# david-cortes/cmfrec

Measured on AMD Instinct MI355X. Metric: ALS rows/sec ((users+items)/iteration time), implicit ALS-CG k=50 fp64, higher is better.
Workload: dtype f64

## Files before the change

### cmfrec_amd/csrc/cg_kernels.hpp

```cpp
#pragma once
#include <hip/hip_runtime.h>
#include <stdint.h>
#include <type_traits>

#include "lanes.hpp"

namespace cmfhip {

constexpr int WAVE = 64;
constexpr int TILE = 64;
constexpr int MAX_W = 8;
#ifndef CMF_CG_WAVES_PER_SIMD
#define CMF_CG_WAVES_PER_SIMD 2
#endif
#ifndef CMF_CG_WAVES_PER_SIMD_F32
#define CMF_CG_WAVES_PER_SIMD_F32 3
#endif
#ifndef CMF_CG_WAVES_PER_SIMD_LOW
#define CMF_CG_WAVES_PER_SIMD_LOW 3
#endif
constexpr int CG_NTSEL_MAX_S = 7;
template <typename T, int W, int NRES_, int NTSEL = 0> constexpr int cg_waves_per_simd()
{
    if (sizeof(T) == 8 && NTSEL == 1 && W <= 8) return CMF_CG_WAVES_PER_SIMD_LOW;
// ... 52 lines not shown
    const T *values;
    const T *bias_sub;
    const T *weights = nullptr;
    const T *wsum = nullptr;
    const int *order;
    const RowDesc *desc;
    int nrows;
    const T *BtB;
    T lam, lam_last;
    int scale_lam, scale_bias_const;
    int max_cg_steps;
    int precond;
    int koff = 0, kc = 0;
    const T *CtC = nullptr;
    const T *UC = nullptr;
    T w_side = 0;
    int rows_with_u = 0;
    int row_first = 0;
    const size_t *indptr2 = nullptr;
    const int *indices2 = nullptr;
    const T *values2 = nullptr;
    const T *C2 = nullptr;
    int *counter = nullptr;
    int p_side = 0, scale_lam_sideinfo = 0;
    const T *Bi = nullptr;
    const T *BiTBi = nullptr;
    int ki = 0;
    T w_imp = 0;
    const T *rconst = nullptr;
    size_t ldr = 0;
    int gx = 0;
#ifdef CMF_CG_DEBUG
    int dbg = 0;
#endif
#ifdef CMF_CG_TICKS
    unsigned long long *ticks = nullptr;
#endif
};
#ifdef CMF_CG_TICKS
#define CMF_TICK() __builtin_amdgcn_s_memtime()
__device__ __forceinline__ void cg_ticks_flush(unsigned long long *t, int slot, unsigned long long wait, unsigned long long pass, unsigned long long rows,
                                               unsigned long long total, int lane)
{
    if (t != nullptr && lane == 0) {
        atomicAdd(t + 4 * slot + 0, wait); atomicAdd(t + 4 * slot + 1, pass); atomicAdd(t + 4 * slot + 2, rows); atomicAdd(t + 4 * slot + 3, total);
    }
// ... 889 lines not shown
{
    static_assert(NE == 4 || NE == 2 || NE == 0, "entries per lane group");
    constexpr bool MIX = NE == 0;
    static_assert(!MIX || CMF_TINY_WAVES_PER_SIMD >= 3, "the mixed launch lives in the dynamically scheduled loop");
    using Tile = typename TinyTile<T, S, (NE == 2) ? 2 : 4>::type;
    constexpr bool GRAM = IMPLICIT || GRAMX;
    extern __shared__ __attribute__((aligned(16))) unsigned char smem_raw[];
    T *G = reinterpret_cast<T *>(smem_raw);
    constexpr bool PV = pass_vector_in_lds<T>();
    __shared__ __attribute__((aligned(16))) T s_pv[PV ? 4 : 1][PV ? 64 : 1];
    const int tid = threadIdx.x;
    const int lane = tid & 63;
    auto short_row = [&](int nnz_) -> bool { return MIX && nnz_ <= 16; };
    auto entry_of = [&](int nnz_) -> int { return (NE == 2 || short_row(nnz_)) ? (lane >> 2) : (lane >> 1); };
    const int k = P.k;
    constexpr bool GREG = tiny_greg<T, GRAM>();
    constexpr int GR = GREG ? gram_rows<T>(S) : 8;
    if (GRAM) {
        stage_gramian<T, S, GR>(G, P.BtB, k, tid, blockDim.x);
        __syncthreads();
    }
    GramRegs<T, GREG ? S : 1, GREG ? GR : 8> greg;
    if constexpr (GREG) greg.load(G, lane);
    const int nwaves = gridDim.x * 4;
    struct Pre { int idx; T x; T a; T g; };
    auto load_desc = [&](int rix_) -> RowDesc {
        RowDesc d; d.row = 0; d.nnz = 0; d.st = 0;
        if (rix_ < P.nrows) d = P.desc[rix_];
        d.row = __builtin_amdgcn_readfirstlane(d.row);
        d.nnz = __builtin_amdgcn_readfirstlane(d.nnz);
        d.st = ((unsigned long long)(unsigned)__builtin_amdgcn_readfirstlane((int)(d.st >> 32)) << 32) |
               (unsigned)__builtin_amdgcn_readfirstlane((int)(d.st & 0xffffffffu));
        return d;
    };
    auto load_pre = [&](const RowDesc &d) -> Pre {
        Pre q; q.idx = 0; q.x = T(0); q.a = T(0); q.g = T(1);
        const int ent = entry_of(d.nnz);
        if (ent < d.nnz) {
            const size_t pos = d.st + (size_t)ent;
            q.idx = P.indices[pos];
            q.x = P.values[pos];
            q.g = entry_weight<T, IMPLICIT>(P, pos);
            if (!IMPLICIT && P.bias_sub != nullptr) q.x -= P.bias_sub[q.idx];
        }
        if (d.nnz > 0 && lane < k) q.a = P.A[(size_t)d.row * P.lda + lane];
        return q;
    };
// ... 47 lines not shown
        if (GRAMX && P.rconst != nullptr && lane < k) r_d += P.rconst[(size_t)d.row * P.ldr + lane];
        if (lane >= k) r_d = T(0);
        T p_d = r_d;
        T r_old = wave_sum(r_d * r_d);
        bool done = (r_old <= (T)1e-12);
        for (int step = 0; step < P.max_cg_steps && !done; step++) {
            T Ap_d = run_pass(p_d, std::integral_constant<int, 1>{});
            Ap_d += lam * p_d;
            if (!IMPLICIT && lam != lam_last && lane == k - 1) Ap_d += (lam_last - lam) * p_d;
            if (lane >= k) Ap_d = T(0);
            T alpha = cg_div(r_old, wave_sum(Ap_d * p_d));
            a_d += alpha * p_d;
            r_d -= alpha * Ap_d;
            T r_new = wave_sum(r_d * r_d);
            if (r_new <= (T)1e-8) done = true;
            else {
                p_d = p_d * cg_div(r_new, r_old) + r_d;
                r_old = r_new;
            }
        }
        if (lane < k) P.A[(size_t)d.row * P.lda + lane] = a_d;
    };

    int rix = blockIdx.x * 4 + (tid >> 6);
#if CMF_TINY_WAVES_PER_SIMD >= 3
    {
        const int cslot = rix % CG_NCOUNTERS;
        int *const my_counter = P.counter + cslot * CG_COUNTER_STRIDE;
        const int cbase = nwaves + cslot;
        auto issue_claim = [&]() -> int {
            int v = 0;
            if (lane == 0) v = atomicAdd(my_counter, 1);
            return v;
        };
        const int c1 = issue_claim(), c2 = issue_claim();
        int rnxt = cbase + CG_NCOUNTERS * __builtin_amdgcn_readfirstlane(c1);
        int rnn = cbase + CG_NCOUNTERS * __builtin_amdgcn_readfirstlane(c2);
        RowDesc d0 = load_desc(rix), d1 = load_desc(rnxt);
        Pre p0 = load_pre(d0);
        Tile tA;
        int pend = issue_claim();
        while (rix < P.nrows) {
            const bool shrt = short_row(d0.nnz);
            if (CMF_DBG(P, 1)) {
                dbg_fill_tile<(NE == 2) ? 2 : 4, S>(tA, (T)(p0.idx & 3) * (T)0.001);
            } else if constexpr (MIX) {
                if (shrt) load_tile2<T, S>(tA, P.B, P.ldb, k, p0.idx, d0.nnz, lane);
// ... 505 lines not shown
```

### cmfrec_amd/csrc/device.hpp

```cpp
#pragma once
#include <hip/hip_runtime.h>
#include <algorithm>
#include <cstdio>
#include <cstdlib>
#include <cstring>
#include <numeric>
#include <string>
#include <vector>

#include "../../include/cmfrec_hip.h"
#include "device_base.hpp"
#include "cg_kernels.hpp"
#include "chol_kernels.hpp"
#include "dense_kernels.hpp"
#include "gram_cg_kernels.hpp"
#include "topn_kernels.hpp"

namespace cmfhip {

constexpr int MAX_DEVICES = 16;
constexpr int NBINS = 6;
constexpr int BIN_VHEAVY = 0;
constexpr int BIN_HEAVY = 1;
constexpr int BIN_MED4 = 2;
// ... 198 lines not shown
            sl_vrow.upload(s_row.data(), s_row.size(), st);
            sl_first.upload(s_first.data(), s_first.size(), st);
            sl_count.upload(s_count.data(), s_count.size(), st);
            row_sl_off.upload(s_off.data(), s_off.size(), st);
            h_row_sl_off = s_off;
            gram_part.alloc((size_t)n_slices * GRAM_PART);
        }
        HIP_CHECK(hipStreamSynchronize(st));
    }
};

struct DeviceInfo {
    int device = 0;
    int num_cus = 256;
    hipStream_t stream = nullptr;
    DevBuf<real_t> cg_gfull, cg_rconst;
    DevBuf<real_t> tile_init;
    DevBuf<int> row_counter;
    DevBuf<real_t> potrs_inv, potrs_tmp;
    DevBuf<real_t> potrs_ref;
    DevBuf<real_t> gemm_ws;
    hipStream_t aux_stream = nullptr;
    hipEvent_t fork_ev = nullptr, join_ev = nullptr;
    hipStream_t eig_stream_ = nullptr;
    hipEvent_t eig_fork = nullptr;
    hipStream_t eig_stream()
    {
        if (!eig_stream_) HIP_CHECK(hipStreamCreateWithFlags(&eig_stream_, hipStreamNonBlocking));
        return eig_stream_;
    }
    mutable bool nonneg_now = false;
    mutable int max_cd_steps = 100;
    mutable real_t l1_now = 0;
    mutable real_t l1_last_now = 0;
    mutable real_t l1_scale = 1;
    DeviceInfo() = default;
    DeviceInfo(const DeviceInfo &) = delete;
    DeviceInfo &operator=(const DeviceInfo &) = delete;
    ~DeviceInfo()
    {
        if (eig_fork) (void)hipEventDestroy(eig_fork);
        if (eig_stream_) (void)hipStreamDestroy(eig_stream_);
        if (fork_ev) (void)hipEventDestroy(fork_ev);
        if (join_ev) (void)hipEventDestroy(join_ev);
        for (int i = 0; i < MAX_BIN_STREAMS; i++) {
            if (bin_join[i]) (void)hipEventDestroy(bin_join[i]);
            if (i > 0 && bin_streams[i]) (void)hipStreamDestroy(bin_streams[i]);
        }
        if (aux_stream) (void)hipStreamDestroy(aux_stream);
        if (stream) (void)hipStreamDestroy(stream);
    }
    void ensure_aux()
    {
        if (aux_stream) return;
        HIP_CHECK(hipStreamCreateWithFlags(&aux_stream, hipStreamNonBlocking));
        HIP_CHECK(hipEventCreateWithFlags(&fork_ev, hipEventDisableTiming));
        HIP_CHECK(hipEventCreateWithFlags(&join_ev, hipEventDisableTiming));
    }
    static constexpr int MAX_BIN_STREAMS = 5;
    hipStream_t bin_streams[MAX_BIN_STREAMS] = {nullptr, nullptr, nullptr, nullptr, nullptr};
    hipEvent_t bin_join[MAX_BIN_STREAMS] = {nullptr, nullptr, nullptr, nullptr, nullptr};
    void ensure_bin_streams(int n)
    {
        ensure_aux();
        bin_streams[0] = aux_stream;
        if (!bin_join[0]) HIP_CHECK(hipEventCreateWithFlags(&bin_join[0], hipEventDisableTiming));
        for (int i = 1; i < n && i < MAX_BIN_STREAMS; i++) {
            if (!bin_streams[i]) HIP_CHECK(hipStreamCreateWithFlags(&bin_streams[i], hipStreamNonBlocking));
            if (!bin_join[i]) HIP_CHECK(hipEventCreateWithFlags(&bin_join[i], hipEventDisableTiming));
        }
    }
};

struct EventPair { hipEvent_t a, b; };
struct BinTimers {
    std::vector<EventPair> ev[NBINS];
    void clear()
    {
        for (auto &v : ev) {
            for (auto &p : v) { (void)hipEventDestroy(p.a); (void)hipEventDestroy(p.b); }
// ... 43 lines not shown
    if (k <= 64) {
        int nblocks = std::max(1, std::min(dev.num_cus * 2, (n + 127) / 128));
        int rpb = (n + nblocks - 1) / nblocks;
        nblocks = (n + rpb - 1) / rpb;
        if (nblocks < 1) nblocks = 1;
        size_t need = (size_t)nblocks * k * k;
        if (ws.partial.n < need) ws.partial.alloc(need);
        const int rem = (sizeof(real_t) == 8 && k > 48 && k <= 52) ? k - 48 : 0;
        switch (rem) {
#define CMF_GRAM_REM(R) case R: hipLaunchKernelGGL((gram_mfma_partial_kernel<real_t, R>), dim3(nblocks), dim3(256), 0, dev.stream, B, ldb, n, k, rpb, ws.partial.ptr); break;
            CMF_GRAM_REM(1) CMF_GRAM_REM(2) CMF_GRAM_REM(3) CMF_GRAM_REM(4)
#undef CMF_GRAM_REM
            default: hipLaunchKernelGGL((gram_mfma_partial_kernel<real_t, 0>), dim3(nblocks), dim3(256), 0, dev.stream, B, ldb, n, k, rpb, ws.partial.ptr); break;
        }
        hipLaunchKernelGGL(gram_reduce_kernel<real_t>, dim3((k * k + GRAM_RED_ENT - 1) / GRAM_RED_ENT), dim3(256), 0, dev.stream,
                           ws.partial.ptr, nblocks, k * k, out, scale, add_diag, k);
    } else {
        launch_gemm<true>(dev, k, k, n, scale, B, ldb, B, ldb, out, (size_t)k);
        if (add_diag != 0)
            hipLaunchKernelGGL(add_diag_kernel<real_t>, dim3((k + 255) / 256), dim3(256), 0, dev.stream, out, k, 0, k, add_diag);
    }
    HIP_CHECK(hipGetLastError());
}

struct CgCall {
    real_t *A; size_t lda;
    const real_t *B; size_t ldb;
    int k;
    const real_t *bias_sub;
    const real_t *BtB;
    real_t lam, lam_last;
    bool scale_lam, scale_bias_const;
    int max_cg_steps;
    bool implicit;
    bool precond = false;
    int koff = 0, kc = 0;
    const real_t *CtC = nullptr, *UC = nullptr;
    real_t w_side = 0;
    int rows_with_u = 0, p_side = 0;
    bool scale_lam_sideinfo = false;
    const SparseShard *X2 = nullptr;
    const real_t *C2 = nullptr;
    const real_t *Bi = nullptr, *BiTBi = nullptr;
    int ki = 0;
    real_t w_imp = 0;
    const real_t *gsum = nullptr;
    int skip_first = 0;
    const real_t *Gx = nullptr, *rconst_x = nullptr;
    size_t ldr_x = 0;
    const real_t *values_override = nullptr, *weights_override = nullptr;
    bool gx_all_rows = false;
    const real_t *wsum_override = nullptr;
};

enum class CgVariant { Auto, Generic };
CgVariant cg_variant_from_env();

constexpr int NCOUNTER_SETS = 2 * NBINS + 2;
constexpr size_t ROW_COUNTER_INTS = 64 + (size_t)NCOUNTER_SETS * CG_NCOUNTERS * CG_COUNTER_STRIDE;
inline size_t cg_counter_offset(int bin) { return 64 + (size_t)bin * CG_NCOUNTERS * CG_COUNTER_STRIDE; }

__global__ void __launch_bounds__(256) poison_lds_kernel(int words)
{
    extern __shared__ unsigned int poison_words[];
    volatile unsigned int *w = poison_words;
    for (int e = threadIdx.x; e < words; e += 256) w[e] = 0xFFFFFFFFu;
}
inline void poison_lds(hipStream_t st, int num_cus)
{
    if (!switches().poison_lds) return;
    constexpr int BYTES = 80 * 1024;
    static thread_local bool attr_set = false;
    if (!attr_set) {
        HIP_CHECK(hipFuncSetAttribute((const void *)poison_lds_kernel, hipFuncAttributeMaxDynamicSharedMemorySize, BYTES));
        attr_set = true;
// ... 20 lines not shown
    constexpr int threads = 64 * W * RPB;
    size_t smem = (((IMPLICIT || GRAMX) ? (size_t)gram_elems<real_t>(S) : 0) + (size_t)RPB * 2 * W * 64) * sizeof(real_t);
    auto kern = cg_rows_kernel<real_t, S, IMPLICIT, W, RPB, GRAMX, NRES_, NTSEL>;
    static thread_local int bpc_dev[MAX_DEVICES] = {0};
    int &blocks_per_cu = bpc_dev[std::min(std::max(dev.device, 0), MAX_DEVICES - 1)];
    if (blocks_per_cu == 0) {
        if (smem > 48 * 1024)
            HIP_CHECK(hipFuncSetAttribute((const void *)kern, hipFuncAttributeMaxDynamicSharedMemorySize, (int)smem));
        int nb = 0;
        HIP_CHECK(hipOccupancyMaxActiveBlocksPerMultiprocessor(&nb, kern, threads, smem));
        blocks_per_cu = std::max(1, nb);
    }
    int teams_needed = (count + RPB - 1) / RPB;
    int grid = std::min(teams_needed, dev.num_cus * blocks_per_cu);
    hipLaunchKernelGGL(kern, dim3(grid), dim3(threads), smem, st, P);
    HIP_CHECK(hipGetLastError());
    if (tm) {
        HIP_CHECK(hipEventRecord(ev.b, st));
        tm->ev[bin].push_back(ev);
    }
}

template <int S, bool IMPLICIT, bool GRAMX = false>
inline void launch_cg_tiny(const DeviceInfo &dev, CgParams<real_t> P, int first, int count, BinTimers *tm, hipStream_t st, int n_gt16)
{
    if (count <= 0) return;
    EventPair ev{nullptr, nullptr};
    if (tm) {
        HIP_CHECK(hipEventCreate(&ev.a));
        HIP_CHECK(hipEventCreate(&ev.b));
        HIP_CHECK(hipEventRecord(ev.a, st));
    }
    poison_lds(st, dev.num_cus);
    constexpr bool tiny16_on = true;
    const int count_le16 = std::min(count, std::max(0, first + count - std::max(first, n_gt16)));
    size_t smem = ((IMPLICIT || GRAMX) ? (size_t)gram_elems<real_t>(S) : 0) * sizeof(real_t);
    const int di = std::min(std::max(dev.device, 0), MAX_DEVICES - 1);
    CgParams<real_t> P1 = P;
    P1.order += first;
    P1.desc += first;
    P1.nrows = count;
    P1.counter = dev.row_counter.ptr + cg_counter_offset(BIN_TINY);
    {
        const bool mixed = tiny16_on && count_le16 > 0;
        auto kern = mixed ? cg_rows_tiny_kernel<real_t, S, IMPLICIT, GRAMX, 0> : cg_rows_tiny_kernel<real_t, S, IMPLICIT, GRAMX, 4>;
        static thread_local int bpc_dev[MAX_DEVICES][2] = {{0}};
        int &blocks_per_cu = bpc_dev[di][mixed ? 1 : 0];
        if (blocks_per_cu == 0) {
            int nb = 0;
            HIP_CHECK(hipOccupancyMaxActiveBlocksPerMultiprocessor(&nb, kern, 256, smem));
            blocks_per_cu = std::max(1, nb);
        }
        const int grid = std::min((count + 3) / 4, dev.num_cus * blocks_per_cu);
        hipLaunchKernelGGL(kern, dim3(grid), dim3(256), smem, st, P1);
    }
    HIP_CHECK(hipGetLastError());
    if (tm) {
        HIP_CHECK(hipEventRecord(ev.b, st));
        tm->ev[BIN_TINY].push_back(ev);
    }
}

void launch_gram_wave(dim3 grid, hipStream_t st, const CgParams<real_t> &P, const GramParams<real_t> &G, bool implicit, int rem);

template <bool GRAMX>
inline bool vh_takes_gram(int k, const SparseShard &X)
{
    if (GRAMX || k > 16 * GRAM_NTT) return false;
    return (switches().vh != 0) ? switches().vh == 2 : X.prefer_gram((size_t)k * sizeof(real_t));
}

template <int S, bool IMPLICIT, bool GRAMX = false>
inline void launch_cg_vheavy(const DeviceInfo &dev_, CgParams<real_t> P, const SparseShard &X, BinTimers *tm, hipStream_t st)
{
    const int nvh = X.bin_rows[BIN_VHEAVY];
    if (nvh <= 0) return;
    struct { hipStream_t stream; int num_cus; } dev{st, dev_.num_cus};
    EventPair ev{nullptr, nullptr};
    if (tm) {
        HIP_CHECK(hipEventCreate(&ev.a));
        HIP_CHECK(hipEventCreate(&ev.b));
        HIP_CHECK(hipEventRecord(ev.a, dev.stream));
    }
    if (vh_takes_gram<GRAMX>(P.k, X)) {
        GramParams<real_t> G;
        G.sl_vrow = X.sl_vrow.ptr; G.sl_first = X.sl_first.ptr; G.sl_count = X.sl_count.ptr; G.row_sl_off = X.row_sl_off.ptr;
        G.part = X.gram_part.ptr; G.n_slices = X.n_slices; G.nvh = nvh;
        P.nrows = nvh;
#ifdef CMF_CG_DEBUG
        if (switches().debug_ticks) {
            static unsigned long long *d_t = nullptr;
            unsigned long long h[4];
            if (d_t == nullptr) { HIP_CHECK(hipMalloc((void **)&d_t, sizeof(h))); HIP_CHECK(hipMemset(d_t, 0, sizeof(h))); }
            else {
                HIP_CHECK(hipDeviceSynchronize());
                HIP_CHECK(hipMemcpy(h, d_t, sizeof(h), hipMemcpyDeviceToHost));
                if (h[1] > 0)
                    fprintf(stderr, "gram_wave: %.0f ticks per wave, %llu waves, %llu slices, %llu nnz: %.1f ticks per nnz and wave\n",
                            (double)h[0] / h[1], h[1], h[2], h[3], (double)h[0] / (double)h[3]);
                HIP_CHECK(hipMemset(d_t, 0, sizeof(h)));
            }
            G.ticks = d_t;
        }
#endif
        poison_lds(dev.stream, dev.num_cus);
        const bool slice_kernel = switches().gram_slice;
        if (slice_kernel)
            hipLaunchKernelGGL((gram_slice_kernel<real_t, IMPLICIT>), dim3(std::min(X.n_slices, dev.num_cus * 2)), dim3(64 * GRAM_NW), 0,
                           dev.stream, P, G);
        else {
            const dim3 gw(std::min((X.n_slices + 3) / 4, dev.num_cus * 4));
            const int rem = (sizeof(real_t) == 8) ? P.k - 16 * (GRAM_NTT - 1) : 0;
            launch_gram_wave(gw, dev.stream, P, G, IMPLICIT, rem);
        }
        poison_lds(dev.stream, dev.num_cus);
        hipLaunchKernelGGL((gram_cg_kernel<real_t, IMPLICIT>), dim3(std::min(nvh, dev.num_cus * 8)), dim3(256), 0, dev.stream, P, G);
        HIP_CHECK(hipGetLastError());
        if (tm) {
            HIP_CHECK(hipEventRecord(ev.b, dev.stream));
            tm->ev[BIN_VHEAVY].push_back(ev);
        }
        return;
    }
    VhState<real_t> V;
    V.r = X.vh_r.ptr; V.p = X.vh_p.ptr; V.r_old = X.vh_r_old.ptr; V.done = X.vh_done.ptr; V.part = X.vh_part.ptr;
    V.chunk_row = X.vh_chunk_row.ptr; V.chunk_start = X.vh_chunk_start.ptr; V.chunk_cnt = X.vh_chunk_cnt.ptr;
    V.chunk_off = X.vh_chunk_off.ptr; V.launch = X.vh_launch.ptr; V.work = X.vh_work.ptr;
    V.nvh = nvh; V.nchunks = X.n_chunks; V.nlaunch = X.n_launch;
    P.nrows = nvh;
    poison_lds(dev.stream, dev.num_cus);
    const dim3 gp(X.n_launch), bp(64 * VH_CHUNK_TILES), gu(nvh), bu(64 * VH_UPD_WAVES);
    hipLaunchKernelGGL((vh_pass_kernel<real_t, S, IMPLICIT, 0>), gp, bp, 0, dev.stream, P, V);
    hipLaunchKernelGGL((vh_update_kernel<real_t, IMPLICIT, 0, GRAMX>), gu, bu, 0, dev.stream, P, V);
    for (int step = 0; step < P.max_cg_steps; step++) {
        hipLaunchKernelGGL((vh_pass_kernel<real_t, S, IMPLICIT, 1>), gp, bp, 0, dev.stream, P, V);
        hipLaunchKernelGGL((vh_update_kernel<real_t, IMPLICIT, 1, GRAMX>), gu, bu, 0, dev.stream, P, V);
    }
// ... 38 lines not shown
inline void launch_cg_any_bin(const DeviceInfo &dev, const CgParams<real_t> &P, const SparseShard &X, BinTimers *tm, int bin, hipStream_t st)
{
    const int first = X.bin_first[bin], count = X.bin_rows[bin];
    switch (bin) {
        case BIN_HEAVY:
#ifdef CMFREC_HIP_FLOAT
            {
                const int n_long8 = std::min(count, std::max(0, X.n_gt512 - first));
                EventPair ev{nullptr, nullptr};
                if (tm) { HIP_CHECK(hipEventCreate(&ev.a)); HIP_CHECK(hipEventCreate(&ev.b)); HIP_CHECK(hipEventRecord(ev.a, st)); }
                launch_cg_bin<S, IMPLICIT, 8, 1, GRAMX>(dev, P, first, n_long8, nullptr, bin, st);
                launch_cg_bin<S, IMPLICIT, 4, 1, GRAMX, 2>(dev, P, first + n_long8, count - n_long8, nullptr, bin, st, NBINS);
                if (tm) { HIP_CHECK(hipEventRecord(ev.b, st)); tm->ev[bin].push_back(ev); }
                break;
            }
#endif
            launch_cg_bin_by_tile<S, IMPLICIT, 8, 1, GRAMX>(dev, P, X, first, count, tm, bin, st); break;
        case BIN_MED4: launch_cg_bin_by_tile<S, IMPLICIT, 4, 1, GRAMX>(dev, P, X, first, count, tm, bin, st); break;
        case BIN_MED2: launch_cg_bin_by_tile<S, IMPLICIT, 2, 1, GRAMX>(dev, P, X, first, count, tm, bin, st); break;
        default: launch_cg_bin_by_tile<S, IMPLICIT, 1, 4, GRAMX>(dev, P, X, first, count, tm, bin, st); break;
    }
}

template <int S, bool IMPLICIT, bool GRAMX = false>
inline void launch_cg_S(const DeviceInfo &dev, const CgParams<real_t> &P, const SparseShard &X, BinTimers *tm)
{
    if (dev.row_counter.n < ROW_COUNTER_INTS) const_cast<DeviceInfo &>(dev).row_counter.alloc(ROW_COUNTER_INTS);
    HIP_CHECK(hipMemsetAsync(dev.row_counter.ptr, 0, ROW_COUNTER_INTS * sizeof(int), dev.stream));
    const bool vh_aside = X.bin_rows[BIN_VHEAVY] > 0 && X.vh_runs_aside(dev.num_cus) && !vh_takes_gram<GRAMX>(P.k, X);
    const bool alt = X.is_part;
    DeviceInfo &d = const_cast<DeviceInfo &>(dev);
    const int npar = cg_bin_streams();
    if (npar > 1 && !(vh_aside || alt)) {
        d.ensure_bin_streams(npar - 1);
        hipStream_t ss[DeviceInfo::MAX_BIN_STREAMS + 1];
        ss[0] = dev.stream;
        for (int i = 1; i < npar; i++) ss[i] = d.bin_streams[i - 1];
        HIP_CHECK(hipEventRecord(d.fork_ev, dev.stream));
        for (int i = 1; i < npar; i++) HIP_CHECK(hipStreamWaitEvent(ss[i], d.fork_ev, 0));
        static const double row_equiv[NBINS] = {0.0, 126.0, 7.0, 7.0, 0.0, 11.5};
        double cost[NBINS], load[DeviceInfo::MAX_BIN_STREAMS + 1] = {0, 0, 0, 0, 0, 0};
        int order_b[NBINS];
        for (int b = 0; b < NBINS; b++) {
            cost[b] = (double)X.bin_nnz[b] + row_equiv[b] * (double)X.bin_rows[b];
            order_b[b] = b;
        }
        std::sort(order_b, order_b + NBINS, [&](int a, int b2) { return cost[a] > cost[b2]; });
        for (int q = 0; q < NBINS; q++) {
            const int b = order_b[q];
            if (X.bin_rows[b] <= 0) continue;
            int si = 0;
            for (int i = 1; i < npar; i++) if (load[i] < load[si]) si = i;
            load[si] += cost[b];
            if (b == BIN_VHEAVY) launch_cg_vheavy<S, IMPLICIT, GRAMX>(dev, P, X, tm, ss[si]);
            else if (b == BIN_TINY) launch_cg_tiny<S, IMPLICIT, GRAMX>(dev, P, X.bin_first[BIN_TINY], X.bin_rows[BIN_TINY], tm, ss[si], X.n_gt16);
            else launch_cg_any_bin<S, IMPLICIT, GRAMX>(dev, P, X, tm, b, ss[si]);
        }
        for (int i = 1; i < npar; i++) {
            HIP_CHECK(hipEventRecord(d.bin_join[i - 1], ss[i]));
            HIP_CHECK(hipStreamWaitEvent(dev.stream, d.bin_join[i - 1], 0));
        }
        return;
    }
    if (vh_aside || alt) {
        d.ensure_aux();
        HIP_CHECK(hipEventRecord(d.fork_ev, dev.stream));
        HIP_CHECK(hipStreamWaitEvent(d.aux_stream, d.fork_ev, 0));
// ... 51 lines not shown

inline int launch_cg(const DeviceInfo &dev, const CgCall &c, const SparseShard &X, BinTimers *tm = nullptr)
{
    CgParams<real_t> P;
    P.A = c.A; P.lda = c.lda; P.B = c.B; P.ldb = c.ldb; P.k = c.k;
    P.indptr = X.p.ptr; P.indices = X.i.ptr; P.values = X.v.ptr;
    P.bias_sub = c.bias_sub; P.order = X.order.ptr; P.desc = X.desc.ptr; P.nrows = 0; P.BtB = c.BtB;
    if (!c.implicit && X.weighted()) { P.weights = X.w.ptr; P.wsum = X.wsum.ptr; }
    P.lam = c.lam; P.lam_last = c.lam_last;
    P.scale_lam = c.scale_lam; P.scale_bias_const = c.scale_bias_const;
    P.max_cg_steps = c.max_cg_steps;
    P.precond = c.precond ? 1 : 0;
    P.koff = c.koff; P.kc = c.kc; P.CtC = c.CtC; P.UC = c.UC; P.w_side = c.w_side;
    P.rows_with_u = c.rows_with_u; P.p_side = c.p_side; P.scale_lam_sideinfo = c.scale_lam_sideinfo ? 1 : 0;
    if (c.X2) { P.indptr2 = c.X2->p.ptr; P.indices2 = c.X2->i.ptr; P.values2 = c.X2->v.ptr; P.C2 = c.C2; }
    P.Bi = c.Bi; P.BiTBi = c.BiTBi; P.ki = c.ki; P.w_imp = c.w_imp;
#ifdef CMF_CG_DEBUG
    P.dbg = switches().debug_skip;
#endif
#ifdef CMF_CG_TICKS
    P.ticks = cg_ticks_buffer();
#endif
    const int S = (c.k + 7) / 8;
    if (c.values_override != nullptr) P.values = c.values_override;
    if (c.weights_override != nullptr) { P.weights = c.weights_override; P.wsum = X.wsum_naz.ptr; }
    if (c.wsum_override != nullptr) P.wsum = c.wsum_override;
    if (c.Gx != nullptr && (c.kc > 0 || c.X2 != nullptr || c.Bi != nullptr)) {
        if (c.implicit || c.skip_first != 0) {
            g_last_error = "cmfrec_hip: block CG with a shared matrix: the explicit model";
            return 2;
        }
        P.BtB = c.Gx; P.rconst = c.rconst_x; P.ldr = c.ldr_x; P.gx = c.gx_all_rows ? 2 : 1;
        const int NFb = (c.koff + c.k + 63) / 64;
        switch (NFb) {
            case 1: launch_cg_generic<1, false>(dev, P, X, 0, true); return 0;
            case 2: launch_cg_generic<2, false>(dev, P, X, 0, true); return 0;
            case 3: launch_cg_generic<3, false>(dev, P, X, 0, true); return 0;
            default: break;
        }
        g_last_error = "cmfrec_hip: block CG with a shared matrix: at most 192 unknowns per row";
        return 2;
    }
    if (c.Gx != nullptr && c.precond) {
        if (c.implicit || c.kc > 0 || c.Bi != nullptr || c.koff != 0 || c.skip_first != 0 || c.X2 != nullptr) {
            g_last_error = "cmfrec_hip: preconditioned CG with a shared matrix: plain explicit rows";
            return 2;
// ... 42 lines not shown
            CMF_BCASE(1) CMF_BCASE(2) CMF_BCASE(3) CMF_BCASE(4)
            CMF_BCASE(5) CMF_BCASE(6) CMF_BCASE(7) CMF_BCASE(8)
        }
#undef CMF_BCASE
        if (X.nrows > X.n_nonempty) {
            CgParams<real_t> Pe = P;
            Pe.BtB = c.BtB; Pe.rconst = nullptr;
            Pe.row_first = X.n_nonempty; Pe.nrows = X.nrows;
            const int cnt = X.nrows - X.n_nonempty;
            const int NFe = (c.koff + c.k + 63) / 64;
            const int grid = std::min((cnt + 3) / 4, dev.num_cus * 8);
            switch (NFe) {
                case 1: hipLaunchKernelGGL((cg_rows_generic_kernel<real_t, 1, false, 1>), dim3(grid), dim3(256), 0, dev.stream, Pe); break;
                default: hipLaunchKernelGGL((cg_rows_generic_kernel<real_t, 2, false, 1>), dim3(grid), dim3(256), 0, dev.stream, Pe); break;
            }
        }
        HIP_CHECK(hipGetLastError());
        return 0;
    }
    const bool generic = cg_variant_from_env() == CgVariant::Generic || S > 8 || c.precond || c.kc > 0 || c.Bi != nullptr || c.skip_first > 0;
    if (!generic) {
#define CMF_CASE(SS)                                                        \
    case SS:                                                                \
        if (c.implicit) launch_cg_S<SS, true>(dev, P, X, tm);               \
        else            launch_cg_S<SS, false>(dev, P, X, tm);              \
        return 0;
        switch (S) {
            CMF_CASE(1) CMF_CASE(2) CMF_CASE(3) CMF_CASE(4)
            CMF_CASE(5) CMF_CASE(6) CMF_CASE(7) CMF_CASE(8)
        }
#undef CMF_CASE
    }
    const int NF = (c.koff + c.k + 63) / 64;
#define CMF_GCASE(NN)                                                       \
    case NN:                                                                \
        if (c.implicit) launch_cg_generic<NN, true>(dev, P, X, c.skip_first);  \
        else            launch_cg_generic<NN, false>(dev, P, X, c.skip_first); \
        return 0;
    switch (NF) {
        CMF_GCASE(1) CMF_GCASE(2) CMF_GCASE(3) CMF_GCASE(4) CMF_GCASE(5)
    }
#undef CMF_GCASE
    g_last_error = "cmfrec_hip: CG path supports k <= 320 per solved matrix";
    return 2;
}

}
```

### cmfrec_amd/csrc/device_base.hpp

```cpp
#pragma once
#include <hip/hip_runtime.h>
#include <cstdio>
#include <cstdlib>
#include <cstring>
#include <functional>
#include <new>
#include <string>

#include "../../include/cmfrec_hip.h"

namespace cmfhip {

extern thread_local std::string g_last_error;
extern thread_local int g_last_rc;

struct HipError {
    int code;
};

inline void hip_check(hipError_t e, const char *what, const char *file, int line)
{
    if (e == hipSuccess) return;
    char buf[512];
    snprintf(buf, sizeof buf, "cmfrec_hip: %s failed: %s (%s:%d)", what, hipGetErrorString(e), file, line);
// ... 1 lines not shown
    fprintf(stderr, "%s\n", buf);
    throw HipError{e == hipErrorOutOfMemory ? 1 : 4};
}
#define HIP_CHECK(x) ::cmfhip::hip_check((x), #x, __FILE__, __LINE__)

inline int guarded(const std::function<int()> &f)
{
    try {
        return f();
    } catch (const HipError &e) {
        return e.code;
    } catch (const std::bad_alloc &) {
        g_last_error = "cmfrec_hip: host out of memory";
        return 1;
    }
}

struct Switches {
    bool poison_lds = false;
    int vh_min = 0;
    int vh = 0;
    bool gram_slice = false;
    int bins_par = 2;
    bool nt_split = true;
    bool cg_generic = false;
    int chol = 0;
    int parts_coop = 1;
    int chol_wg = 2;
    int gramk = -1;
    int gramk_batch = 0;
    int lowrank = -1;
    bool topn_wide = false;
    int topn_tiles = 0;
    bool eig_jacobi = false;
    int debug_skip = 0;
    bool debug_ticks = false;
    void reload()
    {
        auto str = [](const char *n) -> const char * { const char *v = getenv(n); return (v != nullptr && v[0] != 0) ? v : nullptr; };
        auto num = [&](const char *n, int dflt) -> int { const char *v = str(n); return v ? atoi(v) : dflt; };
        poison_lds = str("CMFREC_HIP_POISON_LDS") != nullptr;
        vh_min = num("CMFREC_HIP_VH_MIN", 0);
        const char *v = str("CMFREC_HIP_VH");
        vh = !v ? 0 : strcmp(v, "stream") == 0 ? 1 : strcmp(v, "gram") == 0 ? 2 : 1;
        v = str("CMFREC_HIP_GRAM_KERNEL"); gram_slice = v && strcmp(v, "slice") == 0;
        bins_par = num("CMFREC_HIP_BINS_PAR", 2);
        nt_split = num("CMFREC_HIP_NT_SPLIT", 1) != 0;
        v = str("CMFREC_HIP_CG_KERNEL"); cg_generic = v && strcmp(v, "generic") == 0;
        v = str("CMFREC_HIP_CHOL"); chol = !v ? 0 : strcmp(v, "rows") == 0 ? 1 : strcmp(v, "noslices") == 0 ? 2 : 0;
        parts_coop = num("CMFREC_HIP_PARTS_COOP", 1);
        chol_wg = num("CMFREC_HIP_CHOL_WG", 2);
        if (chol_wg == 1) chol_wg = 2;
        gramk = num("CMFREC_HIP_GRAMK", -1);
        gramk_batch = num("CMFREC_HIP_GRAMK_BATCH", 0);
        lowrank = num("CMFREC_HIP_LOWRANK", -1);
        v = str("CMFREC_HIP_TOPN"); topn_wide = v && strcmp(v, "wide") == 0;
        topn_tiles = num("CMFREC_HIP_TOPN_TILES", 0);
        v = str("CMFREC_HIP_EIG"); eig_jacobi = v && strcmp(v, "jacobi") == 0;
        debug_skip = num("CMFREC_HIP_CG_SKIP", num("CMFREC_HIP_CHOL_SKIP", num("CMFREC_HIP_WAVE_SKIP", 0)));
        debug_ticks = str("CMFREC_HIP_GRAM_TICKS") != nullptr || str("CMFREC_HIP_CHOL_TICKS") != nullptr;
    }
};
inline Switches &switches_mut() { static Switches sw; static bool first = (sw.reload(), true); (void)first; return sw; }
inline const Switches &switches() { return switches_mut(); }

template <typename T>
struct DevBuf {
    T *ptr = nullptr;
    size_t n = 0;
// ... 41 lines not shown
```

### cmfrec_amd/csrc/session.hip

```cpp
#include "device.hpp"
#include "coo_device.hpp"
#include "chol_wave_kernels.hpp"
#include "gramk_kernels.hpp"
#include "lowrank_kernels.hpp"
#include "eig_kernels.hpp"
#include "gram_cg_wide_kernels.hpp"
#include "side_zeros_kernels.hpp"
#include <dlfcn.h>
#include <functional>
#include <memory>
#include <new>

namespace cmfhip {

thread_local std::string g_last_error;
thread_local int g_last_rc = 0;

CgVariant cg_variant_from_env() { return switches().cg_generic ? CgVariant::Generic : CgVariant::Auto; }

inline dim3 grid1d(size_t n, int block = 256) { return dim3((unsigned)((n + block - 1) / block)); }
hipError_t launch_chol_wg8(int num_cus, bool border, int waves_per_row, hipStream_t st, const CholParams<real_t> &W, const RowDesc *desc, const CholSlices<real_t> &SL);
hipError_t launch_chol_parts_coop(int num_cus, bool border, int depth, hipStream_t st, const CholParams<real_t> &W, const RowDesc *desc, const CholSlices<real_t> &SL);

struct CholCall {
// ... 2097 lines not shown
        launch_gram(dev, s->gws, v.Cm, (size_t)kc, p_self, kc, s->ctc.ptr, (real_t)1, (real_t)0);
        side_times(dev, v.Um_blk, local_u, kc, p_self, (real_t)1, v.Cm, v.uc, (size_t)kc);
        CgCall c = block_cg_call(sbc);
        const int local_u_main = m.implicit ? local_u : std::min(local_u, local_x);
        c.CtC = s->ctc.ptr; c.UC = v.uc; c.rows_with_u = local_u_main;
        add_implicit_term_cg(c);
        int rc = launch_cg_any(dev, c, X, nullptr);
        if (rc) return rc;
        return solve_sideinfo_only_rows(s, v, false, local_u_main, local_u - local_u_main);
    }
    if (m.implicit && p_self > 0) {
        const int kt = k_side_self + kk;
        launch_gram(dev, s->gws, oppx, ld_opp, rows_opp, kk, s->gram.ptr, (real_t)1, lam_self);
        hipLaunchKernelGGL(betbe_base_kernel<real_t>, grid1d(kt * kt), dim3(256), 0, st, s->gram.ptr, kk, k_side_self, lam_self,
                           s->betbe.ptr);
        launch_gram(dev, s->gws, v.Cm, (size_t)kc, p_self, kc, s->ctc.ptr, w, (real_t)0);
        if (X.nrows) HIP_CHECK(hipMemsetAsync(self_blk, 0, (size_t)X.nrows * ld_self * sizeof(real_t), st));
        side_times(dev, v.Um_blk, local_u, kc, p_self, w, v.Cm, self_blk, ld_self);
        CholCall c{self_blk, ld_self, oppx, ld_opp, kt, k_side_self, nullptr, s->ctc.ptr, kc, local_u,
                   p_self, lam_self, lam_last_self, false, false, false, CHOL_COLLECTIVE_IMPLICIT, s->betbe.ptr};
        return launch_chol(dev, c, &X);
    }
    if (m.implicit) {
        if (part <= 0)
            launch_gram(dev, s->gws, oppx, ld_opp, rows_opp, kk, s->gram.ptr, (real_t)1, chol ? lam_self : (real_t)0);
        if (chol) {
            if (X.nrows) HIP_CHECK(hipMemsetAsync(self_blk, 0, (size_t)X.nrows * ld_self * sizeof(real_t), st));
            CholCall c{self_blk + k_side_self, ld_self, oppx, ld_opp, kk, 0, nullptr,
                       s->gram.ptr, 0, 0, 0, lam_self, lam_last_self, false, false, false, CHOL_IMPLICIT};
            return launch_chol(dev, c, &X);
        }
        CgCall c{self_blk + k_side_self, ld_self, oppx, ld_opp, kk, nullptr, s->gram.ptr,
                 lam_self, lam_last_self, false, false, m.max_cg_steps, true, (bool)m.precondition_cg};
        return launch_cg_any(dev, c, X, v.bins);
    }

    fill_fixed_bias_column(s, v);
    HIP_CHECK(hipGetLastError());
    const real_t *bias_sub = v.bias;
    const int ksolve = v.ks, kt = v.kt;
    const real_t *Fi = chol ? v.Fi : nullptr;
    if (Fi != nullptr) {
        launch_implicit_gram(s, v, rows_opp, true, false);
        hipLaunchKernelGGL(embed_block_kernel<real_t>, grid1d(kt * kt), dim3(256), 0, st, s->bitbi.ptr, kk, k_side_self,
                           kt, s->bitbi_full.ptr);
        HIP_CHECK(hipGetLastError());
    }
    auto add_implicit_term = [&](CholCall &c) {
        if (Fi == nullptr) return;
        c.Mfull = s->bitbi_full.ptr;
        if (part < 0 && launch_gsum(s, v, Fi, (size_t)kk, kk, s->grhs.ptr, X.nrows)) {
            add_implicit_rhs(s, v, self_blk, ld_self);
            c.rhs_prefilled_all = true;
            return;
        }
        c.X2 = &X; c.values2 = s->ones.ptr; c.B2 = Fi; c.ldb2 = (size_t)kk; c.kc2 = kk; c.koff2 = k_side_self;
// ... 1375 lines not shown
```

Measured before the change: 168.1 million.

## Add two-stream bin plan with balanced bins, split tiny bin, and gram overlap

Adds a new scheduling plan for the implicit CG solve when two bin streams are used. Bins are sorted by cost and split across the two streams, either greedily or by exhaustive balancing. The tiny bin is deferred and split in half across both streams via wave_base offsets so both finish together. The Gramian computation can be deferred so it runs beside the very-heavy bin's per-row gram work on the other stream. This targets idle GPU time from unbalanced stream loads and the serial Gramian. In exchange it adds event and stream overhead, and the shared row counter means the split tiny launches must cover disjoint wave ranges correctly.

```diff
diff --git a/cmfrec_amd/csrc/cg_kernels.hpp b/cmfrec_amd/csrc/cg_kernels.hpp
--- a/cmfrec_amd/csrc/cg_kernels.hpp
+++ b/cmfrec_amd/csrc/cg_kernels.hpp
@@ -98,6 +98,7 @@
     const T *values2 = nullptr;
     const T *C2 = nullptr;
     int *counter = nullptr;
+    int wave_base = 0, wave_total = 0;
     int p_side = 0, scale_lam_sideinfo = 0;
     const T *Bi = nullptr;
     const T *BiTBi = nullptr;
@@ -1033,7 +1034,7 @@
     }
     GramRegs<T, GREG ? S : 1, GREG ? GR : 8> greg;
     if constexpr (GREG) greg.load(G, lane);
-    const int nwaves = gridDim.x * 4;
+    const int nwaves = P.wave_total;
     struct Pre { int idx; T x; T a; T g; };
     auto load_desc = [&](int rix_) -> RowDesc {
         RowDesc d; d.row = 0; d.nnz = 0; d.st = 0;
@@ -1127,7 +1128,7 @@
         if (lane < k) P.A[(size_t)d.row * P.lda + lane] = a_d;
     };
 
-    int rix = blockIdx.x * 4 + (tid >> 6);
+    int rix = P.wave_base + blockIdx.x * 4 + (tid >> 6);
 #if CMF_TINY_WAVES_PER_SIMD >= 3
     {
         const int cslot = rix % CG_NCOUNTERS;
diff --git a/cmfrec_amd/csrc/device.hpp b/cmfrec_amd/csrc/device.hpp
--- a/cmfrec_amd/csrc/device.hpp
+++ b/cmfrec_amd/csrc/device.hpp
@@ -244,6 +244,7 @@
     DevBuf<real_t> gemm_ws;
     hipStream_t aux_stream = nullptr;
     hipEvent_t fork_ev = nullptr, join_ev = nullptr;
+    hipEvent_t gram_ev = nullptr;
     hipStream_t eig_stream_ = nullptr;
     hipEvent_t eig_fork = nullptr;
     hipStream_t eig_stream()
@@ -265,6 +266,7 @@
         if (eig_stream_) (void)hipStreamDestroy(eig_stream_);
         if (fork_ev) (void)hipEventDestroy(fork_ev);
         if (join_ev) (void)hipEventDestroy(join_ev);
+        if (gram_ev) (void)hipEventDestroy(gram_ev);
         for (int i = 0; i < MAX_BIN_STREAMS; i++) {
             if (bin_join[i]) (void)hipEventDestroy(bin_join[i]);
             if (i > 0 && bin_streams[i]) (void)hipStreamDestroy(bin_streams[i]);
@@ -278,6 +280,7 @@
         HIP_CHECK(hipStreamCreateWithFlags(&aux_stream, hipStreamNonBlocking));
         HIP_CHECK(hipEventCreateWithFlags(&fork_ev, hipEventDisableTiming));
         HIP_CHECK(hipEventCreateWithFlags(&join_ev, hipEventDisableTiming));
+        HIP_CHECK(hipEventCreateWithFlags(&gram_ev, hipEventDisableTiming));
     }
     static constexpr int MAX_BIN_STREAMS = 5;
     hipStream_t bin_streams[MAX_BIN_STREAMS] = {nullptr, nullptr, nullptr, nullptr, nullptr};
@@ -367,6 +370,15 @@
     }
     HIP_CHECK(hipGetLastError());
 }
+
+struct GramJob {
+    GramWorkspace *ws;
+    const real_t *B; size_t ldb;
+    int n, k;
+    real_t *out;
+    real_t scale, add_diag;
+    void run(const DeviceInfo &dev) const { launch_gram(dev, *ws, B, ldb, n, k, out, scale, add_diag); }
+};
 
 struct CgCall {
     real_t *A; size_t lda;
@@ -396,6 +408,7 @@
     const real_t *values_override = nullptr, *weights_override = nullptr;
     bool gx_all_rows = false;
     const real_t *wsum_override = nullptr;
+    const GramJob *gram_job = nullptr;
 };
 
 enum class CgVariant { Auto, Generic };
@@ -462,16 +475,18 @@
 }
 
 template <int S, bool IMPLICIT, bool GRAMX = false>
-inline void launch_cg_tiny(const DeviceInfo &dev, CgParams<real_t> P, int first, int count, BinTimers *tm, hipStream_t st, int n_gt16)
-{
-    if (count <= 0) return;
+inline bool launch_cg_tiny(const DeviceInfo &dev, CgParams<real_t> P, int first, int count, BinTimers *tm, hipStream_t st, int n_gt16,
+                           int tail_part = 0)
+{
+    if (count <= 0) return false;
+    if (tail_part < 0) tm = nullptr;
     EventPair ev{nullptr, nullptr};
     if (tm) {
         HIP_CHECK(hipEventCreate(&ev.a));
         HIP_CHECK(hipEventCreate(&ev.b));
         HIP_CHECK(hipEventRecord(ev.a, st));
     }
-    poison_lds(st, dev.num_cus);
+    if (tail_part >= 0) poison_lds(st, dev.num_cus);
     constexpr bool tiny16_on = true;
     const int count_le16 = std::min(count, std::max(0, first + count - std::max(first, n_gt16)));
     size_t smem = ((IMPLICIT || GRAMX) ? (size_t)gram_elems<real_t>(S) : 0) * sizeof(real_t);
@@ -491,7 +506,15 @@
             HIP_CHECK(hipOccupancyMaxActiveBlocksPerMultiprocessor(&nb, kern, 256, smem));
             blocks_per_cu = std::max(1, nb);
         }
-        const int grid = std::min((count + 3) / 4, dev.num_cus * blocks_per_cu);
+        const int full = dev.num_cus * blocks_per_cu;
+        int grid = std::min((count + 3) / 4, full);
+        if (tail_part < 0) return CMF_TINY_WAVES_PER_SIMD >= 3 && full >= 2 && count >= full * 4;
+        P1.wave_total = grid * 4;
+        if (tail_part > 0) {
+            const int g1 = (grid + 1) / 2;
+            P1.wave_base = (tail_part == 1) ? 0 : g1 * 4;
+            grid = (tail_part == 1) ? g1 : grid - g1;
+        }
         hipLaunchKernelGGL(kern, dim3(grid), dim3(256), smem, st, P1);
     }
     HIP_CHECK(hipGetLastError());
@@ -499,6 +522,7 @@
         HIP_CHECK(hipEventRecord(ev.b, st));
         tm->ev[BIN_TINY].push_back(ev);
     }
+    return true;
 }
 
 void launch_gram_wave(dim3 grid, hipStream_t st, const CgParams<real_t> &P, const GramParams<real_t> &G, bool implicit, int rem);
@@ -510,8 +534,9 @@
     return (switches().vh != 0) ? switches().vh == 2 : X.prefer_gram((size_t)k * sizeof(real_t));
 }
 
-template <int S, bool IMPLICIT, bool GRAMX = false>
-inline void launch_cg_vheavy(const DeviceInfo &dev_, CgParams<real_t> P, const SparseShard &X, BinTimers *tm, hipStream_t st)
+struct NoHook { void operator()() const {} };
+template <int S, bool IMPLICIT, bool GRAMX = false, typename Hook = NoHook>
+inline void launch_cg_vheavy(const DeviceInfo &dev_, CgParams<real_t> P, const SparseShard &X, BinTimers *tm, hipStream_t st, Hook before_cg = Hook())
 {
     const int nvh = X.bin_rows[BIN_VHEAVY];
     if (nvh <= 0) return;
@@ -553,6 +578,7 @@
             const int rem = (sizeof(real_t) == 8) ? P.k - 16 * (GRAM_NTT - 1) : 0;
             launch_gram_wave(gw, dev.stream, P, G, IMPLICIT, rem);
         }
+        before_cg();
         poison_lds(dev.stream, dev.num_cus);
         hipLaunchKernelGGL((gram_cg_kernel<real_t, IMPLICIT>), dim3(std::min(nvh, dev.num_cus * 8)), dim3(256), 0, dev.stream, P, G);
         HIP_CHECK(hipGetLastError());
@@ -637,15 +663,84 @@
     }
 }
 
+inline double cg_bin_cost(const SparseShard &X, int b)
+{
+    static const double row_equiv[NBINS] = {0.0, 126.0, 7.0, 7.0, 0.0, 11.5};
+    return (double)X.bin_nnz[b] + row_equiv[b] * (double)X.bin_rows[b];
+}
+
 template <int S, bool IMPLICIT, bool GRAMX = false>
-inline void launch_cg_S(const DeviceInfo &dev, const CgParams<real_t> &P, const SparseShard &X, BinTimers *tm)
-{
-    if (dev.row_counter.n < ROW_COUNTER_INTS) const_cast<DeviceInfo &>(dev).row_counter.alloc(ROW_COUNTER_INTS);
-    HIP_CHECK(hipMemsetAsync(dev.row_counter.ptr, 0, ROW_COUNTER_INTS * sizeof(int), dev.stream));
+inline void launch_cg_S(const DeviceInfo &dev, const CgParams<real_t> &P, const SparseShard &X, BinTimers *tm, const GramJob *gram_job = nullptr)
+{
     const bool vh_aside = X.bin_rows[BIN_VHEAVY] > 0 && X.vh_runs_aside(dev.num_cus) && !vh_takes_gram<GRAMX>(P.k, X);
     const bool alt = X.is_part;
     DeviceInfo &d = const_cast<DeviceInfo &>(dev);
     const int npar = cg_bin_streams();
+    const int plan = (npar == 2 && !(vh_aside || alt)) ? switches().plan : 0;
+    int seq[NBINS], nseq = 0;
+    for (int b = 0; b < NBINS; b++) if (X.bin_rows[b] > 0) seq[nseq++] = b;
+    if (!(plan & 1)) std::stable_sort(seq, seq + nseq, [&](int a, int b2) { return cg_bin_cost(X, a) > cg_bin_cost(X, b2); });
+    const bool gram_beside = gram_job != nullptr && (plan & 4) && nseq > 0 && seq[0] == BIN_VHEAVY && vh_takes_gram<GRAMX>(P.k, X);
+    if (gram_job != nullptr && !gram_beside) gram_job->run(dev);
+    if (dev.row_counter.n < ROW_COUNTER_INTS) d.row_counter.alloc(ROW_COUNTER_INTS);
+    HIP_CHECK(hipMemsetAsync(dev.row_counter.ptr, 0, ROW_COUNTER_INTS * sizeof(int), dev.stream));
+    if (plan != 0) {
+        d.ensure_bin_streams(1);
+        hipStream_t ss[2] = {dev.stream, d.bin_streams[0]};
+        HIP_CHECK(hipEventRecord(d.fork_ev, dev.stream));
+        HIP_CHECK(hipStreamWaitEvent(ss[1], d.fork_ev, 0));
+        const int tiny_first = X.bin_first[BIN_TINY], tiny_rows = X.bin_rows[BIN_TINY];
+        const bool tiny_last = (plan & 2) && tiny_rows > 0;
+        const bool tiny_shared = tiny_last && launch_cg_tiny<S, IMPLICIT, GRAMX>(dev, P, tiny_first, tiny_rows, nullptr, nullptr, X.n_gt16, -1);
+        if (tiny_last) nseq = (int)(std::remove(seq, seq + nseq, BIN_TINY) - seq);
+        int side[NBINS] = {0, 0, 0, 0, 0, 0};
+        double load[2] = {0, 0};
+        if (plan & 1) {
+            double total = 0, best = -1;
+            int best_mask = 0;
+            for (int i = 0; i < nseq; i++) total += cg_bin_cost(X, seq[i]);
+            for (int mask = 0; nseq > 0 && mask < (1 << (nseq - 1)); mask++) {
+                double l1 = 0;
+                for (int i = 1; i < nseq; i++) if ((mask >> (i - 1)) & 1) l1 += cg_bin_cost(X, seq[i]);
+                const double diff = std::fabs(total - 2 * l1);
+                if (best < 0 || diff < best) { best = diff; best_mask = mask; }
+            }
+            for (int i = 1; i < nseq; i++) side[seq[i]] = (best_mask >> (i - 1)) & 1;
+        } else {
+            double l[2] = {0, 0};
+            for (int i = 0; i < nseq; i++) {
+                const int si = l[1] < l[0] ? 1 : 0;
+                side[seq[i]] = si;
+                l[si] += cg_bin_cost(X, seq[i]);
+            }
+        }
+        if (gram_beside && side[BIN_VHEAVY] == 0) for (int i = 0; i < nseq; i++) side[seq[i]] ^= 1;
+        for (int i = 0; i < nseq; i++) load[side[seq[i]]] += cg_bin_cost(X, seq[i]);
+        for (int i = 0; i < nseq; i++) {
+            const int b = seq[i];
+            hipStream_t st = ss[side[b]];
+            if (b == BIN_VHEAVY && gram_beside)
+                launch_cg_vheavy<S, IMPLICIT, GRAMX>(dev, P, X, tm, st, [&]() {
+                    gram_job->run(dev);
+                    HIP_CHECK(hipEventRecord(d.gram_ev, dev.stream));
+                    HIP_CHECK(hipStreamWaitEvent(st, d.gram_ev, 0));
+                });
+            else if (b == BIN_VHEAVY) launch_cg_vheavy<S, IMPLICIT, GRAMX>(dev, P, X, tm, st);
+            else if (b == BIN_TINY) launch_cg_tiny<S, IMPLICIT, GRAMX>(dev, P, tiny_first, tiny_rows, tm, st, X.n_gt16);
+            else launch_cg_any_bin<S, IMPLICIT, GRAMX>(dev, P, X, tm, b, st);
+        }
+        const int lighter = load[1] < load[0] ? 1 : 0;
+        EventPair ev{nullptr, nullptr};
+        if (tiny_shared) {
+            if (tm) { HIP_CHECK(hipEventCreate(&ev.a)); HIP_CHECK(hipEventCreate(&ev.b)); HIP_CHECK(hipEventRecord(ev.a, ss[lighter])); }
+            launch_cg_tiny<S, IMPLICIT, GRAMX>(dev, P, tiny_first, tiny_rows, nullptr, ss[lighter], X.n_gt16, 1);
+            launch_cg_tiny<S, IMPLICIT, GRAMX>(dev, P, tiny_first, tiny_rows, nullptr, ss[1 - lighter], X.n_gt16, 2);
+        } else if (tiny_last) launch_cg_tiny<S, IMPLICIT, GRAMX>(dev, P, tiny_first, tiny_rows, tm, ss[lighter], X.n_gt16);
+        HIP_CHECK(hipEventRecord(d.bin_join[0], ss[1]));
+        HIP_CHECK(hipStreamWaitEvent(dev.stream, d.bin_join[0], 0));
+        if (tiny_shared && tm) { HIP_CHECK(hipEventRecord(ev.b, dev.stream)); tm->ev[BIN_TINY].push_back(ev); }
+        return;
+    }
     if (npar > 1 && !(vh_aside || alt)) {
         d.ensure_bin_streams(npar - 1);
         hipStream_t ss[DeviceInfo::MAX_BIN_STREAMS + 1];
@@ -653,11 +748,10 @@
         for (int i = 1; i < npar; i++) ss[i] = d.bin_streams[i - 1];
         HIP_CHECK(hipEventRecord(d.fork_ev, dev.stream));
         for (int i = 1; i < npar; i++) HIP_CHECK(hipStreamWaitEvent(ss[i], d.fork_ev, 0));
-        static const double row_equiv[NBINS] = {0.0, 126.0, 7.0, 7.0, 0.0, 11.5};
         double cost[NBINS], load[DeviceInfo::MAX_BIN_STREAMS + 1] = {0, 0, 0, 0, 0, 0};
         int order_b[NBINS];
         for (int b = 0; b < NBINS; b++) {
-            cost[b] = (double)X.bin_nnz[b] + row_equiv[b] * (double)X.bin_rows[b];
+            cost[b] = cg_bin_cost(X, b);
             order_b[b] = b;
         }
         std::sort(order_b, order_b + NBINS, [&](int a, int b2) { return cost[a] > cost[b2]; });
@@ -755,6 +849,9 @@
     P.ticks = cg_ticks_buffer();
 #endif
     const int S = (c.k + 7) / 8;
+    const bool plain_tiled = c.Gx == nullptr && c.kc == 0 && c.Bi == nullptr && c.skip_first == 0 && !c.precond && S <= 8 &&
+                             cg_variant_from_env() != CgVariant::Generic;
+    if (c.gram_job != nullptr && !plain_tiled) c.gram_job->run(dev);
     if (c.values_override != nullptr) P.values = c.values_override;
     if (c.weights_override != nullptr) { P.weights = c.weights_override; P.wsum = X.wsum_naz.ptr; }
     if (c.wsum_override != nullptr) P.wsum = c.wsum_override;
@@ -843,8 +940,8 @@
     if (!generic) {
 #define CMF_CASE(SS)                                                        \
     case SS:                                                                \
-        if (c.implicit) launch_cg_S<SS, true>(dev, P, X, tm);               \
-        else            launch_cg_S<SS, false>(dev, P, X, tm);              \
+        if (c.implicit) launch_cg_S<SS, true>(dev, P, X, tm, c.gram_job);   \
+        else            launch_cg_S<SS, false>(dev, P, X, tm, c.gram_job);  \
         return 0;
         switch (S) {
             CMF_CASE(1) CMF_CASE(2) CMF_CASE(3) CMF_CASE(4)
diff --git a/cmfrec_amd/csrc/device_base.hpp b/cmfrec_amd/csrc/device_base.hpp
--- a/cmfrec_amd/csrc/device_base.hpp
+++ b/cmfrec_amd/csrc/device_base.hpp
@@ -47,6 +47,7 @@
     int vh = 0;
     bool gram_slice = false;
     int bins_par = 2;
+    int plan = 7;
     bool nt_split = true;
     bool cg_generic = false;
     int chol = 0;
@@ -70,6 +71,7 @@
         vh = !v ? 0 : strcmp(v, "stream") == 0 ? 1 : strcmp(v, "gram") == 0 ? 2 : 1;
         v = str("CMFREC_HIP_GRAM_KERNEL"); gram_slice = v && strcmp(v, "slice") == 0;
         bins_par = num("CMFREC_HIP_BINS_PAR", 2);
+        plan = num("CMFREC_HIP_PLAN", 7) & 7;
         nt_split = num("CMFREC_HIP_NT_SPLIT", 1) != 0;
         v = str("CMFREC_HIP_CG_KERNEL"); cg_generic = v && strcmp(v, "generic") == 0;
         v = str("CMFREC_HIP_CHOL"); chol = !v ? 0 : strcmp(v, "rows") == 0 ? 1 : strcmp(v, "noslices") == 0 ? 2 : 0;
diff --git a/cmfrec_amd/csrc/session.hip b/cmfrec_amd/csrc/session.hip
--- a/cmfrec_amd/csrc/session.hip
+++ b/cmfrec_amd/csrc/session.hip
@@ -2143,8 +2143,9 @@
         return launch_chol(dev, c, &X);
     }
     if (m.implicit) {
-        if (part <= 0)
-            launch_gram(dev, s->gws, oppx, ld_opp, rows_opp, kk, s->gram.ptr, (real_t)1, chol ? lam_self : (real_t)0);
+        const GramJob gj{&s->gws, oppx, ld_opp, rows_opp, kk, s->gram.ptr, (real_t)1, chol ? lam_self : (real_t)0};
+        const bool gram_in_cg = !chol && part < 0;
+        if (part <= 0 && !gram_in_cg) gj.run(dev);
         if (chol) {
             if (X.nrows) HIP_CHECK(hipMemsetAsync(self_blk, 0, (size_t)X.nrows * ld_self * sizeof(real_t), st));
             CholCall c{self_blk + k_side_self, ld_self, oppx, ld_opp, kk, 0, nullptr,
@@ -2153,6 +2154,7 @@
         }
         CgCall c{self_blk + k_side_self, ld_self, oppx, ld_opp, kk, nullptr, s->gram.ptr,
                  lam_self, lam_last_self, false, false, m.max_cg_steps, true, (bool)m.precondition_cg};
+        if (gram_in_cg) c.gram_job = &gj;
         return launch_cg_any(dev, c, X, v.bins);
     }
 
```

Result: no change. 168.9 million, median of 6 (+0.5%).
